# hikvision-research/ProbabilisticTeacher

Measured on AMD Instinct MI355X. Metric: teacher-student train-step img/s at 1333x800, higher is better.
Workload: dtype f32; 1 GPU; BASELINE configs[2]: final_c2f.yaml (K=8) full teacher+student+EMA step, per-GPU 16 labelled + 16 unlabelled synthetic 1333x800 images, BURN_UP_STEP=0, random init; global_batch=32, parallelism=dp1

## Files before the change

probabilisticteacher_amd/csrc/nms.hip:

```cpp
#include "common.h"

namespace {

typedef unsigned long long u64;

__device__ __forceinline__ int seg_count(const int32_t* __restrict__ seg, const int32_t* __restrict__ cnt, int img)
{
    const int cap = seg[img + 1] - seg[img];
    return cnt ? min(cap, cnt[img]) : cap;
}

__global__ __launch_bounds__(64) void nms_mask_kernel(const float* __restrict__ boxes,
                                                      const int32_t* __restrict__ seg,
                                                      const int32_t* __restrict__ cnt, float thr, int words,
                                                      int64_t max_count, u64* __restrict__ mask)
{
    const int cb = blockIdx.x, rb = blockIdx.y, img = blockIdx.z;
    if (cb < rb) return;
    const int beg = seg[img], n = seg_count(seg, cnt, img);
    if (rb * 64 >= n || cb * 64 >= n) return;
    __shared__ float4 cbox[64];
    __shared__ float carea[64];
    const int t = threadIdx.x;
    const int cj = cb * 64 + t;
    if (cj < n) {
        const float4 b = reinterpret_cast<const float4*>(boxes)[beg + cj];
        cbox[t] = b;
        carea[t] = (b.z - b.x) * (b.w - b.y);
    }
    __syncthreads();
    const int i = rb * 64 + t;
    if (i >= n) return;
    const float4 a = reinterpret_cast<const float4*>(boxes)[beg + i];
    const float aarea = (a.z - a.x) * (a.w - a.y);
    const int lim = min(64, n - cb * 64);
    u64 bits = 0;
    const int start = (cb == rb) ? t + 1 : 0;
    constexpr float HI = 1.f + 0x1p-20f, LO = 1.f - 0x1p-20f;
    for (int k = start; k < lim; ++k) {
        const float4 b = cbox[k];
        const float xx1 = fmaxf(a.x, b.x), yy1 = fmaxf(a.y, b.y);
        const float xx2 = fminf(a.z, b.z), yy2 = fminf(a.w, b.w);
        float w = xx2 - xx1, h = yy2 - yy1;
        w = w < 0.f ? 0.f : w;
        h = h < 0.f ? 0.f : h;
        const float inter = w * h;
        const float uni = aarea + carea[k] - inter;
        const float p = thr * uni;
        bool sup;
        if (uni > 0.f && p >= 1.17549435e-38f && inter > p * HI) sup = true;
        else if (uni > 0.f && p >= 1.17549435e-38f && inter < p * LO) sup = false;
        else sup = inter / uni > thr;
        if (sup) bits |= 1ull << k;
    }
    mask[((size_t)img * max_count + i) * words + cb] = bits;
}

constexpr int SCAN_THREADS = 256;

__global__ __launch_bounds__(SCAN_THREADS) void nms_scan_kernel(const u64* __restrict__ mask, const int32_t* __restrict__ seg,
                                                                const int32_t* __restrict__ cnt, int words, int64_t max_count,
                                                                int max_keep, int32_t* __restrict__ keep,
                                                                int32_t* __restrict__ keep_count)
{
    extern __shared__ u64 removed[];
    __shared__ u64 kept_s;
    __shared__ int count_s;
    const int img = blockIdx.x, tid = threadIdx.x, lane = tid & 63;
    const int wave = __builtin_amdgcn_readfirstlane(tid >> 6);
    const int n = seg_count(seg, cnt, img);
    const u64* M = mask + (size_t)img * max_count * words;
    for (int w = tid; w < words; w += SCAN_THREADS) removed[w] = 0;
    if (tid == 0) count_s = 0;
    __syncthreads();
    int count = 0;
    const int chunks = (n + 63) / 64;
    u64 diag_next = (wave == 0 && lane < n) ? M[(size_t)lane * words] : 0;
    for (int c = 0; c < chunks; ++c) {
        if (wave == 0) {
            const int row = c * 64 + lane;
            const u64 diag = diag_next;
            if (c + 1 < chunks) {
                const int rn = row + 64;
                diag_next = (rn < n) ? M[(size_t)rn * words + c + 1] : 0;
            }
            u64 cur = removed[c];
            if (c == chunks - 1 && (n & 63)) cur |= ~0ull << (n & 63);
            u64 alive = ~(((u64)(unsigned)__builtin_amdgcn_readfirstlane((int)(unsigned)(cur >> 32)) << 32) |
                          (u64)(unsigned)__builtin_amdgcn_readfirstlane((int)(unsigned)cur));
            u64 kept = 0;
            const unsigned dlo = (unsigned)diag, dhi = (unsigned)(diag >> 32);
            while (alive) {
                const int i = __builtin_ctzll(alive);
                kept |= 1ull << i;
                const u64 di = ((u64)(unsigned)__builtin_amdgcn_readlane((int)dhi, i) << 32) |
                               (u64)(unsigned)__builtin_amdgcn_readlane((int)dlo, i);
                alive &= ~(di | (1ull << i));
            }
            if ((kept >> lane) & 1ull) {
                const int pos = count + __popcll(kept & ((1ull << lane) - 1ull));
                if (pos < max_keep) keep[(size_t)img * max_keep + pos] = row;
            }
            if (lane == 0) {
                kept_s = kept;
                count_s = count + __popcll(kept);
            }
        }
        __syncthreads();
        count = count_s;
        if (count >= max_keep) break;
        const unsigned klo = (unsigned)__builtin_amdgcn_readfirstlane((int)(unsigned)kept_s);
        const unsigned khi = (unsigned)__builtin_amdgcn_readfirstlane((int)(unsigned)(kept_s >> 32));
        const u64 kept = ((u64)khi << 32) | klo;
        for (int w = c + 1 + tid; w < chunks; w += SCAN_THREADS) {
            u64 acc = removed[w];
            const u64* Mw = M + (size_t)c * 64 * words + w;
            u64 k = kept;
            while (k) {
                u64 v[16];
#pragma unroll
                for (int j = 0; j < 16; ++j) {
                    if (k) {
                        const int i = __builtin_ctzll(k);
                        k &= k - 1;
                        v[j] = Mw[(size_t)i * words];
                    } else v[j] = 0ull;
                }
#pragma unroll
                for (int j = 0; j < 16; ++j) acc |= v[j];
            }
            removed[w] = acc;
        }
        __syncthreads();
    }
    if (tid == 0) keep_count[img] = count < max_keep ? count : max_keep;
}

}

extern "C" {

int64_t ptmi_nms_ws_bytes(int64_t max_count, int nimg)
{
    const int64_t words = (max_count + 63) / 64;
    return (int64_t)nimg * max_count * words * 8;
}

int ptmi_nms_batched(const float* boxes, const int32_t* seg_offsets, const int32_t* seg_counts, int nimg,
                     int64_t max_count, float thr, int max_keep, int32_t* keep_out, int32_t* keep_count, void* ws,
                     ptmi_stream_t s)
{
    PTMI_CHECK_ARG(seg_offsets && keep_out && keep_count && nimg > 0 && max_count >= 0 && max_keep > 0,
                   "nms_batched: bad args");
    PTMI_CHECK_ARG(max_count == 0 || (boxes && ws), "nms_batched: boxes / workspace missing");
    hipStream_t st = (hipStream_t)s;
    if (max_count == 0) {
        hipError_t e = hipMemsetAsync(keep_count, 0, sizeof(int32_t) * (size_t)nimg, st);
        if (e != hipSuccess) { ptmi_set_error("nms_batched: memset failed"); return -2; }
        return 0;
    }
    const int words = (int)((max_count + 63) / 64);
    PTMI_CHECK_ARG((size_t)words * 8 <= 64 * 1024, "nms_batched: max_count %lld too large", (long long)max_count);
    dim3 grid(words, words, nimg);
    hipLaunchKernelGGL(nms_mask_kernel, grid, dim3(64), 0, st, boxes, seg_offsets, seg_counts, thr, words, max_count,
                       reinterpret_cast<u64*>(ws));
    PTMI_LAUNCH_CHECK("nms_mask");
    hipLaunchKernelGGL(nms_scan_kernel, dim3(nimg), dim3(SCAN_THREADS), (size_t)words * 8, st, reinterpret_cast<const u64*>(ws),
                       seg_offsets, seg_counts, words, max_count, max_keep, keep_out, keep_count);
    PTMI_LAUNCH_CHECK("nms_scan");
    return 0;
}

}
```

Measured before the change: 98.92 img/s.

## Restructure batched NMS into banded mask and scan passes with early exit

Replaces the full N×N pairwise suppression mask with a loop over 1024-box bands. Each band computes only the intra-band upper-triangle mask plus suppression from already-kept boxes, which are OR-reduced into a global removed bitmap via atomics. A per-image done flag lets later bands skip work once max_keep is reached. This is meant to cut the quadratic mask computation and memory when few boxes are kept. The cost is more kernel launches per call, one mask-plus-scan pair per band, and extra atomic traffic.

```diff
diff --git a/probabilisticteacher_amd/csrc/nms.hip b/probabilisticteacher_amd/csrc/nms.hip
--- a/probabilisticteacher_amd/csrc/nms.hip
+++ b/probabilisticteacher_amd/csrc/nms.hip
@@ -3,6 +3,9 @@
 namespace {
 
 typedef unsigned long long u64;
+
+constexpr int BAND = 1024;
+constexpr int BAND_WORDS = BAND / 64;
 
 __device__ __forceinline__ int seg_count(const int32_t* __restrict__ seg, const int32_t* __restrict__ cnt, int img)
 {
@@ -10,18 +13,36 @@
     return cnt ? min(cap, cnt[img]) : cap;
 }
 
-__global__ __launch_bounds__(64) void nms_mask_kernel(const float* __restrict__ boxes,
-                                                      const int32_t* __restrict__ seg,
-                                                      const int32_t* __restrict__ cnt, float thr, int words,
-                                                      int64_t max_count, u64* __restrict__ mask)
-{
-    const int cb = blockIdx.x, rb = blockIdx.y, img = blockIdx.z;
-    if (cb < rb) return;
+__global__ __launch_bounds__(64) void nms_mask_band_kernel(const float* __restrict__ boxes,
+                                                           const int32_t* __restrict__ seg,
+                                                           const int32_t* __restrict__ cnt, float thr, int words,
+                                                           int64_t max_count, int band, int kept_blocks, int max_keep,
+                                                           const int32_t* keep, const int32_t* count_st,
+                                                           const int32_t* done_st, u64* removed_st, u64* __restrict__ mask)
+{
+    const int cb = band * BAND_WORDS + blockIdx.x, img = blockIdx.z, t = threadIdx.x;
+    if (band > 0 && done_st[img]) return;
     const int beg = seg[img], n = seg_count(seg, cnt, img);
-    if (rb * 64 >= n || cb * 64 >= n) return;
+    if (cb * 64 >= n) return;
+    const bool kept_rows = (int)blockIdx.y < kept_blocks;
+    int i, start = 0;
+    bool valid;
+    if (kept_rows) {
+        const int count = min(count_st[img], max_keep);
+        if ((int)blockIdx.y * 64 >= count) return;
+        const int idx = blockIdx.y * 64 + t;
+        i = idx < count ? keep[(size_t)img * max_keep + idx] : -1;
+        valid = i >= 0 && i < n;
+        if (!valid) i = 0;
+    } else {
+        const int rb = band * BAND_WORDS + ((int)blockIdx.y - kept_blocks);
+        if (cb < rb || rb * 64 >= n) return;
+        i = rb * 64 + t;
+        valid = i < n;
+        if (cb == rb) start = t + 1;
+    }
     __shared__ float4 cbox[64];
     __shared__ float carea[64];
-    const int t = threadIdx.x;
     const int cj = cb * 64 + t;
     if (cj < n) {
         const float4 b = reinterpret_cast<const float4*>(boxes)[beg + cj];
@@ -29,13 +50,11 @@
         carea[t] = (b.z - b.x) * (b.w - b.y);
     }
     __syncthreads();
-    const int i = rb * 64 + t;
-    if (i >= n) return;
+    if (!valid && !kept_rows) return;
     const float4 a = reinterpret_cast<const float4*>(boxes)[beg + i];
     const float aarea = (a.z - a.x) * (a.w - a.y);
     const int lim = min(64, n - cb * 64);
     u64 bits = 0;
-    const int start = (cb == rb) ? t + 1 : 0;
     constexpr float HI = 1.f + 0x1p-20f, LO = 1.f - 0x1p-20f;
     for (int k = start; k < lim; ++k) {
         const float4 b = cbox[k];
@@ -53,38 +72,62 @@
         else sup = inter / uni > thr;
         if (sup) bits |= 1ull << k;
     }
-    mask[((size_t)img * max_count + i) * words + cb] = bits;
+    if (!kept_rows) {
+        mask[((size_t)img * max_count + i) * BAND_WORDS + blockIdx.x] = bits;
+        return;
+    }
+    unsigned lo = valid ? (unsigned)bits : 0u, hi = valid ? (unsigned)(bits >> 32) : 0u;
+#pragma unroll
+    for (int o = 32; o > 0; o >>= 1) {
+        lo |= (unsigned)__shfl_xor((int)lo, o);
+        hi |= (unsigned)__shfl_xor((int)hi, o);
+    }
+    const u64 any = ((u64)hi << 32) | lo;
+    if (t == 0 && any) atomicOr(&removed_st[(size_t)img * words + cb], any);
 }
 
 constexpr int SCAN_THREADS = 256;
-
-__global__ __launch_bounds__(SCAN_THREADS) void nms_scan_kernel(const u64* __restrict__ mask, const int32_t* __restrict__ seg,
-                                                                const int32_t* __restrict__ cnt, int words, int64_t max_count,
-                                                                int max_keep, int32_t* __restrict__ keep,
-                                                                int32_t* __restrict__ keep_count)
-{
-    extern __shared__ u64 removed[];
+constexpr int SLICES = SCAN_THREADS / BAND_WORDS;
+constexpr int SLICE_ROWS = 64 / SLICES;
+static_assert(SLICES * BAND_WORDS == SCAN_THREADS && SLICES * SLICE_ROWS == 64, "scan thread layout");
+
+__global__ __launch_bounds__(SCAN_THREADS) void nms_scan_band_kernel(const u64* __restrict__ mask,
+                                                                     const int32_t* __restrict__ seg,
+                                                                     const int32_t* __restrict__ cnt, int words,
+                                                                     int64_t max_count, int band, int max_keep,
+                                                                     int32_t* __restrict__ keep,
+                                                                     int32_t* __restrict__ keep_count, int32_t* count_st,
+                                                                     int32_t* done_st, u64* removed_st)
+{
+    __shared__ u64 removed[BAND_WORDS];
     __shared__ u64 kept_s;
     __shared__ int count_s;
     const int img = blockIdx.x, tid = threadIdx.x, lane = tid & 63;
+    if (band > 0 && done_st[img]) return;
     const int wave = __builtin_amdgcn_readfirstlane(tid >> 6);
     const int n = seg_count(seg, cnt, img);
-    const u64* M = mask + (size_t)img * max_count * words;
-    for (int w = tid; w < words; w += SCAN_THREADS) removed[w] = 0;
-    if (tid == 0) count_s = 0;
+    const u64* M = mask + (size_t)img * max_count * BAND_WORDS;
+    u64* R = removed_st + (size_t)img * words;
+    int32_t* K = keep + (size_t)img * max_keep;
+    int count = band > 0 ? min(count_st[img], max_keep) : 0;
+    const int chunks = (n + 63) / 64;
+    const int c0 = band * BAND_WORDS, c1 = min(chunks, c0 + BAND_WORDS);
+    if (band == 0)
+        for (int w = BAND_WORDS + tid; w < words; w += SCAN_THREADS) R[w] = 0;
+    if (tid < BAND_WORDS) removed[tid] = (band > 0 && c0 + tid < c1) ? R[c0 + tid] : 0;
+    if (tid == 0) count_s = count;
     __syncthreads();
-    int count = 0;
-    const int chunks = (n + 63) / 64;
-    u64 diag_next = (wave == 0 && lane < n) ? M[(size_t)lane * words] : 0;
-    for (int c = 0; c < chunks; ++c) {
+    const int wl = tid % BAND_WORDS, slice = tid / BAND_WORDS;
+    u64 diag_next = (wave == 0 && c0 < c1 && c0 * 64 + lane < n) ? M[(size_t)(c0 * 64 + lane) * BAND_WORDS] : 0;
+    for (int c = c0; c < c1; ++c) {
         if (wave == 0) {
             const int row = c * 64 + lane;
             const u64 diag = diag_next;
-            if (c + 1 < chunks) {
+            if (c + 1 < c1) {
                 const int rn = row + 64;
-                diag_next = (rn < n) ? M[(size_t)rn * words + c + 1] : 0;
-            }
-            u64 cur = removed[c];
+                diag_next = (rn < n) ? M[(size_t)rn * BAND_WORDS + (c + 1 - c0)] : 0;
+            }
+            u64 cur = removed[c - c0];
             if (c == chunks - 1 && (n & 63)) cur |= ~0ull << (n & 63);
             u64 alive = ~(((u64)(unsigned)__builtin_amdgcn_readfirstlane((int)(unsigned)(cur >> 32)) << 32) |
                           (u64)(unsigned)__builtin_amdgcn_readfirstlane((int)(unsigned)cur));
@@ -99,7 +142,7 @@
             }
             if ((kept >> lane) & 1ull) {
                 const int pos = count + __popcll(kept & ((1ull << lane) - 1ull));
-                if (pos < max_keep) keep[(size_t)img * max_keep + pos] = row;
+                if (pos < max_keep) K[pos] = row;
             }
             if (lane == 0) {
                 kept_s = kept;
@@ -109,31 +152,26 @@
         __syncthreads();
         count = count_s;
         if (count >= max_keep) break;
-        const unsigned klo = (unsigned)__builtin_amdgcn_readfirstlane((int)(unsigned)kept_s);
-        const unsigned khi = (unsigned)__builtin_amdgcn_readfirstlane((int)(unsigned)(kept_s >> 32));
-        const u64 kept = ((u64)khi << 32) | klo;
-        for (int w = c + 1 + tid; w < chunks; w += SCAN_THREADS) {
-            u64 acc = removed[w];
-            const u64* Mw = M + (size_t)c * 64 * words + w;
-            u64 k = kept;
-            while (k) {
-                u64 v[16];
+        const u64 kept = kept_s;
+        const int w = c + 1 + wl;
+        if (w < c1) {
+            const u64* Mw = M + (size_t)c * 64 * BAND_WORDS + (w - c0);
+            u64 acc = 0;
 #pragma unroll
-                for (int j = 0; j < 16; ++j) {
-                    if (k) {
-                        const int i = __builtin_ctzll(k);
-                        k &= k - 1;
-                        v[j] = Mw[(size_t)i * words];
-                    } else v[j] = 0ull;
-                }
-#pragma unroll
-                for (int j = 0; j < 16; ++j) acc |= v[j];
-            }
-            removed[w] = acc;
+            for (int j = 0; j < SLICE_ROWS; ++j) {
+                const int i = slice * SLICE_ROWS + j;
+                if ((kept >> i) & 1ull) acc |= Mw[(size_t)i * BAND_WORDS];
+            }
+            if (acc) atomicOr(&removed[w - c0], acc);
         }
         __syncthreads();
     }
-    if (tid == 0) keep_count[img] = count < max_keep ? count : max_keep;
+    if (tid == 0) {
+        const bool fin = count >= max_keep || c1 >= chunks;
+        done_st[img] = fin ? 1 : 0;
+        count_st[img] = count;
+        if (fin) keep_count[img] = count < max_keep ? count : max_keep;
+    }
 }
 
 }
@@ -143,7 +181,7 @@
 int64_t ptmi_nms_ws_bytes(int64_t max_count, int nimg)
 {
     const int64_t words = (max_count + 63) / 64;
-    return (int64_t)nimg * max_count * words * 8;
+    return (int64_t)nimg * (max_count * BAND_WORDS + words + 1) * 8;
 }
 
 int ptmi_nms_batched(const float* boxes, const int32_t* seg_offsets, const int32_t* seg_counts, int nimg,
@@ -159,15 +197,24 @@
         if (e != hipSuccess) { ptmi_set_error("nms_batched: memset failed"); return -2; }
         return 0;
     }
+    PTMI_CHECK_ARG(max_count < (1ll << 30), "nms_batched: max_count %lld too large", (long long)max_count);
     const int words = (int)((max_count + 63) / 64);
-    PTMI_CHECK_ARG((size_t)words * 8 <= 64 * 1024, "nms_batched: max_count %lld too large", (long long)max_count);
-    dim3 grid(words, words, nimg);
-    hipLaunchKernelGGL(nms_mask_kernel, grid, dim3(64), 0, st, boxes, seg_offsets, seg_counts, thr, words, max_count,
-                       reinterpret_cast<u64*>(ws));
-    PTMI_LAUNCH_CHECK("nms_mask");
-    hipLaunchKernelGGL(nms_scan_kernel, dim3(nimg), dim3(SCAN_THREADS), (size_t)words * 8, st, reinterpret_cast<const u64*>(ws),
-                       seg_offsets, seg_counts, words, max_count, max_keep, keep_out, keep_count);
-    PTMI_LAUNCH_CHECK("nms_scan");
+    u64* mask = reinterpret_cast<u64*>(ws);
+    u64* removed_st = mask + (size_t)nimg * max_count * BAND_WORDS;
+    int32_t* count_st = reinterpret_cast<int32_t*>(removed_st + (size_t)nimg * words);
+    int32_t* done_st = count_st + nimg;
+    const int bands = (int)((max_count + BAND - 1) / BAND);
+    for (int band = 0; band < bands; ++band) {
+        const int64_t before = (int64_t)band * BAND;
+        const int kept_blocks = (int)(((before < max_keep ? before : (int64_t)max_keep) + 63) / 64);
+        hipLaunchKernelGGL(nms_mask_band_kernel, dim3(BAND_WORDS, kept_blocks + BAND_WORDS, nimg), dim3(64), 0, st, boxes,
+                           seg_offsets, seg_counts, thr, words, max_count, band, kept_blocks, max_keep, keep_out, count_st,
+                           done_st, removed_st, mask);
+        PTMI_LAUNCH_CHECK("nms_mask_band");
+        hipLaunchKernelGGL(nms_scan_band_kernel, dim3(nimg), dim3(SCAN_THREADS), 0, st, mask, seg_offsets, seg_counts, words,
+                           max_count, band, max_keep, keep_out, keep_count, count_st, done_st, removed_st);
+        PTMI_LAUNCH_CHECK("nms_scan_band");
+    }
     return 0;
 }
 
```

Measured after the change: 99.40 img/s (median of 4 runs). About the same (+0.5%).
